# val-iisc/Reflecting-Reality

Hardware: AMD Instinct MI355X
Metric: images/sec at 512x512, 50-step DDIM, SD1.5+BrushNet (higher is better)
Workload: dtype bf16; 1 GPU; SD1.5 + BrushNet(6 cond ch) depth-cond inpaint, batch 4x512x512 per GPU, 50-step DDIM, CFG 7.5, VAE encode+decode included, random-init weights, inputs resident on the device; per_gpu_batch=4, global_batch=4, height=512, width=512, denoise_steps=50, parallelism=batch-shard x1 (no collective)

## Files before the change

reflecting-reality_amd/csrc/gemm_conv_kernel.h:

```cpp
#pragma once
#include "mf_common.h"

#include <type_traits>

#ifndef MF_XTAP
#define MF_XTAP 1
#endif
#ifndef MF_AEARLY
#define MF_AEARLY 1
#endif

namespace mfgemm {

static __device__ __attribute__((aligned(16))) unsigned int g_zero_page[16];

#ifdef MF_STAMPS
#define MF_STAMP(slot) do { if (p.stamps) { const int t_ = (int)threadIdx.x; \
    if (t_ == 0) p.stamps[(size_t)blockIdx.x * 32 + (slot)] = __builtin_amdgcn_s_memrealtime(); \
    else if (t_ == (int)blockDim.x - 256) p.stamps[(size_t)blockIdx.x * 32 + 16 + (slot)] = __builtin_amdgcn_s_memrealtime(); } } while (0)
#define MF_STAMP_DRAIN() asm volatile("s_waitcnt vmcnt(0)" ::: "memory")
#define MF_CLK(v) const unsigned long long v = __builtin_amdgcn_s_memtime()
#define MF_SUM(acc, a, b) acc += (b) - (a)
#define MF_PUT(slot, v) do { if (p.stamps) { const int t_ = (int)threadIdx.x; \
    if (t_ == 0) p.stamps[(size_t)blockIdx.x * 32 + (slot)] = (v); \
    else if (t_ == (int)blockDim.x - 256) p.stamps[(size_t)blockIdx.x * 32 + 16 + (slot)] = (v); } } while (0)
#else
#define MF_STAMP(slot) do { } while (0)
#define MF_STAMP_DRAIN() do { } while (0)
#define MF_CLK(v) do { } while (0)
#define MF_SUM(acc, a, b) do { } while (0)
#define MF_PUT(slot, v) do { } while (0)
#endif

struct GemmArgs {
    const char* a0; const char* a1;
    int C0, Ctot;
    int ld0b, ld1b;
    int Hin, Win, Ho, Wo, HoWo, KW, stride, pad_t, pad_l, ups;
    const char* w; int64_t ldw;
    int M, N, K;
    int zdiv; int64_t a_zs_o, a_zs_i, w_zs_o, w_zs_i, o_zs_o, o_zs_i;
    int splitk, kt_per_split, nkt, nz;
    float* ws;
    unsigned* sk_tickets;
    const float* bias; int bias_mode;
    const float* rs; const float* cs; int64_t rs_zs, cs_zs;
    const float* temb; int64_t ld_temb;
    const char* res0; int res0_dt; int64_t ld_res0;
    const char* res1; int res1_dt; int64_t ld_res1;
    int res1_rows;
    float alpha; int act;
    char* out; int out_dt; int64_t ldc;
    int tiles_n, tiles_m, ord_mfast, ord_pw, nblk, vec_ok, fast, dbg_no_res_pre;
    int dbg_epi;
    int pointwise;
    int howo_sh, wo_sh, ho_sh;
    unsigned wfr_magic;
    int epb;
    int epb_sh;
    unsigned* ovf;
    unsigned long long* stamps;
    const float* ln_cs; float ln_eps;
    char* vt_out; int vt_n0, vt_tokens; int64_t vt_ld;
    int nloop;
    float2* gn_part;
    float2* gn_grp; int gn_cpg;
};

__device__ __forceinline__ int div_sh(int x, int d, int sh) { return sh >= 0 ? x >> sh : x / d; }

__device__ __forceinline__ int res1_row(const GemmArgs& p, int m) {
    if (p.res1_rows > 0)
        while (m >= p.res1_rows) m -= p.res1_rows;
    return m;
}

__device__ __forceinline__ void epilogue_store(const GemmArgs& p, int64_t zo, int m, int n, float v, int zq = 0) {
    if (p.rs) v *= p.rs[zq * p.rs_zs + m];
    if (p.cs) v *= p.cs[zq * p.cs_zs + n];
    if (p.bias) v += p.bias_mode ? p.bias[m] : p.bias[n];
    if (p.temb) v += p.temb[(int64_t)div_sh(m, p.HoWo, p.howo_sh) * p.ld_temb + n];
    v *= p.alpha;
    if (p.res0) v += load_as_f32(p.res0, p.res0_dt, (int64_t)m * p.ld_res0 + n);
    if (p.res1) v += load_as_f32(p.res1, p.res1_dt, (int64_t)res1_row(p, m) * p.ld_res1 + n);
    if (p.act == MF_ACT_SILU) v = silu_precise(v);
    store_from_f32(p.out, p.out_dt, zo + (int64_t)m * p.ldc + n, v);
}

template <bool F16 = false>
__device__ __forceinline__ void load8_as_f32(const char* p, int dt, int64_t idx, float* o) {
    if (dt == MF_F32) {
        const float4 a = *reinterpret_cast<const float4*>(p + idx * 4);
        const float4 b = *reinterpret_cast<const float4*>(p + idx * 4 + 16);
        o[0] = a.x; o[1] = a.y; o[2] = a.z; o[3] = a.w; o[4] = b.x; o[5] = b.y; o[6] = b.z; o[7] = b.w;
    } else {
        unpack_h8<F16>(*reinterpret_cast<const uint4*>(p + idx * 2), o);
    }
}

__device__ __forceinline__ void unpack8_bf16(const uint4& u, float* o) {
    o[0] = __uint_as_float(u.x << 16); o[1] = __uint_as_float(u.x & 0xffff0000u);
    o[2] = __uint_as_float(u.y << 16); o[3] = __uint_as_float(u.y & 0xffff0000u);
    o[4] = __uint_as_float(u.z << 16); o[5] = __uint_as_float(u.z & 0xffff0000u);
    o[6] = __uint_as_float(u.w << 16); o[7] = __uint_as_float(u.w & 0xffff0000u);
}

template <bool F16>
__device__ __forceinline__ void epilogue_store8(const GemmArgs& p, int64_t zo, int m, int n, float* v, bool pre = false,
                                                const uint4& q0 = uint4{0, 0, 0, 0}, const uint4& q1 = uint4{0, 0, 0, 0}, int zq = 0,
                                                const char* eb = nullptr, const char* et = nullptr) {
    if (p.rs || p.cs) {
        const float r = p.rs ? p.rs[zq * p.rs_zs + m] : 1.0f;
        float c8[8] = {1, 1, 1, 1, 1, 1, 1, 1};
        if (p.cs) load8_as_f32((const char*)(p.cs + zq * p.cs_zs), MF_F32, n, c8);
#pragma unroll
        for (int j = 0; j < 8; ++j) v[j] *= r * c8[j];
    }
    if (p.bias) {
        if (p.bias_mode) {
            const float b = p.bias[m];
#pragma unroll
            for (int j = 0; j < 8; ++j) v[j] += b;
        } else {
            float b[8];
            if (eb) load8_as_f32(eb, MF_F32, 0, b);
            else load8_as_f32((const char*)p.bias, MF_F32, n, b);
#pragma unroll
            for (int j = 0; j < 8; ++j) v[j] += b[j];
        }
    }
    if (p.temb) {
        float t[8];
        if (et) load8_as_f32(et, MF_F32, 0, t);
        else load8_as_f32((const char*)p.temb, MF_F32, (int64_t)div_sh(m, p.HoWo, p.howo_sh) * p.ld_temb + n, t);
#pragma unroll
        for (int j = 0; j < 8; ++j) v[j] += t[j];
    }
#pragma unroll
    for (int j = 0; j < 8; ++j) v[j] *= p.alpha;
    if (p.res0) {
        float r[8];
        if (pre) unpack_h8<F16>(q0, r);
        else load8_as_f32<F16>(p.res0, p.res0_dt, (int64_t)m * p.ld_res0 + n, r);
#pragma unroll
        for (int j = 0; j < 8; ++j) v[j] += r[j];
    }
    if (p.res1) {
        float r[8];
        if (pre) unpack_h8<F16>(q1, r);
        else load8_as_f32<F16>(p.res1, p.res1_dt, (int64_t)res1_row(p, m) * p.ld_res1 + n, r);
#pragma unroll
        for (int j = 0; j < 8; ++j) v[j] += r[j];
    }
    if (p.act == MF_ACT_SILU) {
#pragma unroll
        for (int j = 0; j < 8; ++j) v[j] = silu_precise(v[j]);
    }
    if (p.act == MF_ACT_GEGLU4) {
        float g[4];
        if (p.out_dt != MF_F32) {
#pragma unroll
            for (int j = 0; j < 4; ++j) {
                const float x = v[4 + j];
                const float z = fabsf(x) * 0.70710678118654752440f;
                const float t = __builtin_amdgcn_rcpf(fmaf(0.3275911f, z, 1.0f));
                const float poly = t * fmaf(t, fmaf(t, fmaf(t, fmaf(t, 1.061405429f, -1.453152027f), 1.421413741f), -0.284496736f), 0.254829592f);
                const float e = 1.0f - poly * __builtin_amdgcn_exp2f(-z * z * 1.44269504088896340736f);
                g[j] = v[j] * (0.5f * x + 0.5f * fabsf(x) * e);
            }
        } else {
#pragma unroll
            for (int j = 0; j < 4; ++j) g[j] = v[j] * (0.5f * v[4 + j] * (1.0f + erff(v[4 + j] * 0.70710678118654752440f)));
        }
        const int64_t o = zo + (int64_t)m * p.ldc + (n >> 1);
        if (p.out_dt == MF_F32) {
            *reinterpret_cast<float4*>(p.out + o * 4) = make_float4(g[0], g[1], g[2], g[3]);
        } else {
            uint2 u;
            u.x = pack_h2<F16>(g[0], g[1]);
            u.y = pack_h2<F16>(g[2], g[3]);
            *reinterpret_cast<uint2*>(p.out + o * 2) = u;
        }
        return;
    }
    const int64_t o = zo + (int64_t)m * p.ldc + n;
    if (p.out_dt == MF_F32) {
        *reinterpret_cast<float4*>(p.out + o * 4) = make_float4(v[0], v[1], v[2], v[3]);
        *reinterpret_cast<float4*>(p.out + o * 4 + 16) = make_float4(v[4], v[5], v[6], v[7]);
    } else {
        *reinterpret_cast<uint4*>(p.out + o * 2) = pack_h8<F16>(v);
    }
}

__device__ __forceinline__ uint4 ld8f_to_bf16(const char* p) {
    const float4 lo = *reinterpret_cast<const float4*>(p);
    const float4 hi = *reinterpret_cast<const float4*>(p + 16);
    uint4 r;
    r.x = pack_bf16x2(lo.x, lo.y);
    r.y = pack_bf16x2(lo.z, lo.w);
    r.z = pack_bf16x2(hi.x, hi.y);
    r.w = pack_bf16x2(hi.z, hi.w);
    return r;
}

typedef __attribute__((address_space(1))) const void* gbl_ptr_t;

__device__ __forceinline__ void dma16(const char* src, char* lds_wave_base) {
    const unsigned lds_off = __builtin_amdgcn_readfirstlane((unsigned)(size_t)(lds_ptr_t)lds_wave_base);
    unsigned keep;
    asm volatile("s_mov_b32 %0, m0\n\ts_mov_b32 m0, %2\n\ts_nop 0\n\tglobal_load_lds_dwordx4 %1, off\n\ts_mov_b32 m0, %0"
                 : "=&s"(keep) : "v"(src), "s"(lds_off) : "memory");
}

template <int DT>
__device__ __forceinline__ f32x4_t mfma16x32(bf16x8_t a, bf16x8_t b, f32x4_t c, int, int, int) {
    if constexpr (DT == MF_F16) return __builtin_amdgcn_mfma_f32_16x16x32_f16(__builtin_bit_cast(f16x8_t, a), __builtin_bit_cast(f16x8_t, b), c, 0, 0, 0);
    else return __builtin_amdgcn_mfma_f32_16x16x32_bf16(a, b, c, 0, 0, 0);
}
template <int DT>
__device__ __forceinline__ f32x16_t mfma32x16(bf16x8_t a, bf16x8_t b, f32x16_t c) {
    if constexpr (DT == MF_F16) return __builtin_amdgcn_mfma_f32_32x32x16_f16(__builtin_bit_cast(f16x8_t, a), __builtin_bit_cast(f16x8_t, b), c, 0, 0, 0);
    else return __builtin_amdgcn_mfma_f32_32x32x16_bf16(a, b, c, 0, 0, 0);
}

#define MF_FX_XT 1
#define MF_FX_EPB 2
#define MF_FX_AE 4
#define MF_FX_ALL 7
#define MF_FX_XQ 8

constexpr int epb_pitch(int bn) { return (bn + 63) / 64 * 64; }
constexpr int epb_off(int bm, int bn, int stages, bool dx, bool ws) {
    return dx ? 2 * (bm + 32) * 128 + (ws ? stages : 2) * bn * 128 : stages * (bm + bn) * 128 + (ws ? bm * 8 : 0);
}
constexpr int epb_nimg(int bm, int bn, int stages, bool dx, bool ws) {
    if (!ws) return 0;
    const int room = 160 * 1024 - epb_off(bm, bn, stages, dx, ws), row = epb_pitch(bn) * 4;
    return room >= 6 * row ? 4 : (room >= 3 * row ? 1 : 0);
}

constexpr int min_waves(int bm, int bn, int stages, int nthr) {
    const int smem = stages * (bm + bn) * 128;
    int blocks = 160 * 1024 / smem;
    if (blocks > 8) blocks = 8;
    int w = blocks * (nthr / 64) / 4;
    return w < 1 ? 1 : (w > 4 ? 4 : w);
}

template <int BM, int BN, int NT_ALL, bool F16>
__device__ __forceinline__ void splitk_combine_tail(const GemmArgs& p, char* smem, int tile_m, int tile_n, int z, int zq, int64_t zo, int t) {
    asm volatile("s_waitcnt vmcnt(0)" ::: "memory");
    __syncthreads();
    unsigned* last_flag = reinterpret_cast<unsigned*>(smem);
    if (t == 0) {
        __builtin_amdgcn_fence(__ATOMIC_RELEASE, "agent");
        asm volatile("s_waitcnt vmcnt(0)" ::: "memory");
        unsigned* tk = p.sk_tickets + ((int64_t)z * p.tiles_m + tile_m) * p.tiles_n + tile_n;
        const unsigned prev = __hip_atomic_fetch_add(tk, 1u, __ATOMIC_RELAXED, __HIP_MEMORY_SCOPE_AGENT);
        const bool last = prev == (unsigned)p.splitk - 1u;
        if (last) {
            __hip_atomic_store(tk, 0u, __ATOMIC_RELAXED, __HIP_MEMORY_SCOPE_AGENT);
            __builtin_amdgcn_fence(__ATOMIC_ACQUIRE, "agent");
            asm volatile("s_waitcnt vmcnt(0)" ::: "memory");
        }
        *last_flag = last ? 1u : 0u;
    }
    __syncthreads();
    if (*last_flag == 0u) return;
    const int m0 = tile_m * BM, n0 = tile_n * BN;
    constexpr int CPR = BN / 8;
    const int64_t mn = (int64_t)p.M * p.N;
    const bool vec = p.vec_ok && (p.N & 3) == 0;
    for (int it = t; it < BM * CPR; it += NT_ALL) {
        const int row = it / CPR, ec = (it - row * CPR) * 8;
        const int m = m0 + row, n = n0 + ec;
        if (m >= p.M || n >= p.N) continue;
        const float* src = p.ws + (int64_t)z * mn + (int64_t)m * p.N + n;
        if (vec && n + 8 <= p.N) {
            float v[8] = {0, 0, 0, 0, 0, 0, 0, 0};
            for (int s = 0; s < p.splitk; ++s) {
                const float4 a = *reinterpret_cast<const float4*>(src + (int64_t)s * p.nz * mn);
                const float4 b = *reinterpret_cast<const float4*>(src + (int64_t)s * p.nz * mn + 4);
                v[0] += a.x; v[1] += a.y; v[2] += a.z; v[3] += a.w; v[4] += b.x; v[5] += b.y; v[6] += b.z; v[7] += b.w;
            }
            epilogue_store8<F16>(p, zo, m, n, v, false, uint4{0, 0, 0, 0}, uint4{0, 0, 0, 0}, zq);
        } else {
            for (int jj = 0; jj < 8 && n + jj < p.N; ++jj) {
                float v = 0.0f;
                for (int s = 0; s < p.splitk; ++s) v += src[(int64_t)s * p.nz * mn + jj];
                epilogue_store(p, zo, m, n + jj, v, zq);
            }
        }
    }
}

template <int DT, int BM, int BN, int WAVES_M, int WAVES_N, bool A_F32, int STAGES, bool DXR = false, bool WPK = false, bool M16 = false,
          bool WS = false, bool P16 = false, bool SKF = false, int FX = 0>
__global__ __launch_bounds__(WAVES_M* WAVES_N * 64 + (WS ? 256 : 0),
                             WS ? (WAVES_M * WAVES_N + 4) / 4 : min_waves(BM + (DXR ? 32 : 0), BN, STAGES, WAVES_M* WAVES_N * 64))
void gemm_conv_kernel(const GemmArgs p) {
    constexpr int NTHR = WAVES_M * WAVES_N * 64;
    constexpr int NSTG = WS ? 256 : NTHR;
    constexpr bool H16 = DT == MF_BF16 || DT == MF_F16;
    static_assert(!WS || ((H16 || (DT == MF_F16X3 && WPK && !M16 && !P16)) && !A_F32 && STAGES == 3),
                  "warp specialisation: bf16 / fp16 (or the parity mode with a pre-split W), LDS-DMA staging, 3-deep ring");
    static_assert(!M16 || (H16 && !A_F32), "the 16x16x32 form is instantiated for bf16 / fp16 only");
    constexpr bool X1 = DT == MF_BF16X1;
    constexpr bool SPLIT = (DT == MF_F16X3 || DT == MF_BF16X3 || X1);
    static_assert(!WPK || (SPLIT && !X1), "a pre-split W operand only exists for the three-MFMA split codes");
    constexpr bool FP8 = (DT == MF_FP8);
    constexpr int ES = H16 ? 2 : (FP8 ? 1 : 4);
    constexpr int AES = A_F32 ? 4 : ES;
    constexpr int VEC = 16 / ES;
    constexpr int BK = 128 / ES;
    constexpr int WM = BM / WAVES_M, WN = BN / WAVES_N;
    static_assert(!P16 || (H16 && !M16 && !A_F32 && (WM == 32 || WM == 64) && WN % 16 == 0), "P16: 16-bit operands, 32- or 64-row wave tiles");
    constexpr int MT = WM / 32, NT = P16 ? 1 : WN / 32;
    constexpr int MT16 = WM / 16, NT16 = WN / 16;
    constexpr int RPP = NSTG / 8;
    constexpr int A_IT = BM / RPP, B_IT = BN / RPP;
    constexpr int STAGE_BYTES = (BM + BN) * 128;
    constexpr int EP_RS = (WN + 4) * 4;
    static_assert(WM % 32 == 0 && (P16 || WN % 32 == 0), "wave tile must be a multiple of 32x32");
    static_assert(BM % RPP == 0 && BN % RPP == 0, "tile rows must be a multiple of the staging pass");
    constexpr int SR = (WAVES_M * WAVES_N * 32 * EP_RS <= STAGES * STAGE_BYTES) ? 32 : 16;
    static_assert(WAVES_M * WAVES_N * SR * EP_RS <= STAGES * STAGE_BYTES, "epilogue slabs must fit in the staging LDS");
    static_assert(STAGES >= 2 && STAGES <= 6, "2 to 6 LDS stages");
    static_assert(!A_F32 || STAGES == 2, "the register-staged path is double buffered");
    static_assert(!A_F32 || DT == MF_BF16, "A_F32 only converts fp32 activations for bf16 compute");

    extern __shared__ __attribute__((aligned(16))) char smem[];
    MF_STAMP(0);

    const bool producer = WS && __builtin_amdgcn_readfirstlane((int)threadIdx.x) >= NTHR;
    const int tid = producer ? (int)threadIdx.x - NTHR : (int)threadIdx.x;
    const int lane = tid & 63;
    const int wave = __builtin_amdgcn_readfirstlane(tid >> 6);
    const int wm = wave / WAVES_N, wn = wave % WAVES_N;
    if constexpr (WS) {
        if ((p.dbg_epi & 16) && !producer) __builtin_amdgcn_s_setprio(1);
        if ((p.dbg_epi & 32) && producer) __builtin_amdgcn_s_setprio(1);
    }

    int bid = blockIdx.x;
// ... 818 lines not shown
                    st_c = st_c == STAGES - 1 ? 0 : st_c + 1;
                    st_i = st_i == STAGES - 1 ? 0 : st_i + 1;
                }
            };
            auto ring_ws = [&](auto issue) {
                if (producer) {
                    int st_i = 0, issued = 0;
                    auto issue_next = [&]() { issue(st_i); st_i = st_i == STAGES - 1 ? 0 : st_i + 1; ++issued; };
                    auto wait_for = [&](int need) {
                        const int newer = issued - 1 - need;
                        static_assert((PF - 1) * G < 64, "vmcnt is a 6-bit counter");
                        if (PF >= 3 && newer >= 2) wait_vmcnt<2 * G>();
                        else if (PF >= 2 && newer == 1) wait_vmcnt<G>();
                        else wait_vmcnt<0>();
                    };
                    const bool lnf = p.ln_cs != nullptr;
                    float ln_s[A_IT], ln_q[A_IT];
#pragma unroll
                    for (int i = 0; i < A_IT; ++i) { ln_s[i] = 0.0f; ln_q[i] = 0.0f; }
                    int st_s = 0;
                    auto ln_tile = [&]() {
                        if constexpr (DT == MF_BF16) {
                            typedef __attribute__((ext_vector_type(2))) __bf16 bf2_t;
                            const bf2_t ones = __builtin_bit_cast(bf2_t, 0x3F803F80u);
                            const char* As = smem + st_s * STAGE_BYTES + tid * 16;
#pragma unroll
                            for (int i = 0; i < A_IT; ++i) {
                                const uint4 u = *reinterpret_cast<const uint4*>(As + i * RPP * 128);
                                const unsigned w4[4] = {u.x, u.y, u.z, u.w};
#pragma unroll
                                for (int e = 0; e < 4; ++e) {
                                    const bf2_t v = __builtin_bit_cast(bf2_t, w4[e]);
                                    ln_s[i] = __builtin_amdgcn_fdot2_f32_bf16(v, ones, ln_s[i], false);
                                    ln_q[i] = __builtin_amdgcn_fdot2_f32_bf16(v, v, ln_q[i], false);
                                }
                            }
                        } else if constexpr (DT == MF_F16) {
                            const char* As = smem + st_s * STAGE_BYTES + tid * 16;
#pragma unroll
                            for (int i = 0; i < A_IT; ++i) {
                                const uint4 u = *reinterpret_cast<const uint4*>(As + i * RPP * 128);
                                const unsigned w4[4] = {u.x, u.y, u.z, u.w};
#pragma unroll
                                for (int e = 0; e < 4; ++e) {
                                    const mf_f16x2_t v = __builtin_bit_cast(mf_f16x2_t, w4[e]);
                                    const float a0 = (float)v[0], a1 = (float)v[1];
                                    ln_s[i] += a0 + a1;
                                    ln_q[i] = fmaf(a0, a0, fmaf(a1, a1, ln_q[i]));
                                }
                            }
                        }
                        st_s = st_s == STAGES - 1 ? 0 : st_s + 1;
                    };
                    for (int k = 0; k < PF && k < nt; ++k) issue_next();
                    wait_for(0);
                    __builtin_amdgcn_s_barrier();
                    MF_STAMP(2);
                    [[maybe_unused]] unsigned long long w_iss = 0, w_vm = 0, w_bar = 0;
                    for (int t = 0; t + 1 < nt; ++t) {
                        MF_CLK(c0);
                        if (t + PF < nt) issue_next();
                        if (lnf) ln_tile();
                        MF_CLK(c1);
                        wait_for(t + 1);
                        MF_CLK(c2);
                        __builtin_amdgcn_s_barrier();
                        MF_CLK(c3);
                        MF_SUM(w_iss, c0, c1); MF_SUM(w_vm, c1, c2); MF_SUM(w_bar, c2, c3);
                    }
                    MF_PUT(13, w_vm); MF_PUT(14, w_bar); MF_PUT(15, w_iss);
                    if (lnf) {
                        ln_tile();
                        float2* lnst = reinterpret_cast<float2*>(smem + STAGES * STAGE_BYTES);
                        const float invk = 1.0f / (float)p.K;
#pragma unroll
                        for (int i = 0; i < A_IT; ++i) {
                            float s1 = ln_s[i], q1 = ln_q[i];
#pragma unroll
                            for (int off = 1; off < 8; off <<= 1) {
                                s1 += __shfl_xor(s1, off, 64);
                                q1 += __shfl_xor(q1, off, 64);
                            }
                            const float mean = s1 * invk;
                            float var = q1 * invk - mean * mean;
                            if (var < 0.0f) var = 0.0f;
                            if ((tid & 7) == 0) lnst[lrow + i * RPP] = make_float2(mean, 1.0f / sqrtf(var + p.ln_eps));
                        }
                    }
                } else {
                    int st_c = 0;
                    __builtin_amdgcn_s_barrier();
                    MF_STAMP(2);
                    if constexpr (XT) {
                        const int arb = wm * WM + ((P16 || M16) ? r16 : frow);
                        auto ld = [&](auto S, auto P) {
                            const char* Ab = smem + st_c * STAGE_BYTES;
                            const char* Bb = Ab + BM * 128 + (wn * WN + ((P16 || M16) ? r16 : frow)) * 128;
                            if constexpr (P16 || M16) xt_load(S, P, Ab, [&](int t) { return arb + t * 16; }, Bb);
                            else xt_load(S, P, Ab, [&](int i) { return arb + i * 32; }, Bb);
                        };
                        xt_loop(ld, [&]() { st_c = st_c == STAGES - 1 ? 0 : st_c + 1; });
                    } else
                    for (int t = 0; t < nt; ++t) {
                        compute(st_c);
                        st_c = st_c == STAGES - 1 ? 0 : st_c + 1;
                        if (t + 1 < nt) __builtin_amdgcn_s_barrier();
                    }
                }
            };
            if constexpr (WS) {
                if (p.fast) {
                    if (producer) fast_init();
                    ring_ws(issue_tile_fast);
                } else {
                    ring_ws(issue_tile);
                }
            } else if (p.fast) {
                fast_init();
                ring(issue_tile_fast);
            } else {
                ring(issue_tile);
            }
        } else {
            load_tile_regs();
            store_tile_regs(0);
            if (nt > 1) load_tile_regs();
            __syncthreads();
            for (int t = 0; t < nt; ++t) {
                compute(t & 1);
                if (t + 1 < nt) {
                    store_tile_regs((t + 1) & 1);
                    if (t + 2 < nt) load_tile_regs();
                }
                __syncthreads();
            }
        }
    }
    MF_STAMP(3);
    if constexpr (EPB_NIMG > 0) {
        if (producer && epb) wait_vmcnt<0>();
    }
    __syncthreads();
    MF_STAMP(4);
    if constexpr (DT == MF_F16X3) mf_raise_if_over(p.ovf, split_amax);

    char* slab = smem + wave * (SR * EP_RS);
    constexpr int CPR = WN / 8;
    constexpr int ITEMS = SR * CPR;
    float* ws = p.splitk > 1 ? p.ws + ((int64_t)ksplit * p.nz + z) * (int64_t)p.M * p.N : nullptr;
    const int64_t zo = zq * p.o_zs_o + zr * p.o_zs_i;
    const bool res_pre = !ws && p.vec_ok && (p.res0 || p.res1) && (!p.res0 || p.res0_dt != MF_F32) &&
                         (!p.res1 || p.res1_dt != MF_F32) && !p.dbg_no_res_pre;
    constexpr int NIT = (ITEMS + 63) / 64;
    if constexpr (WS) {
        constexpr int NCW = WAVES_M * WAVES_N, TW = NCW + 4, NCHUNK = NCW * NIT, MAXC = (NCHUNK + TW - 1) / TW;
        const int g = producer ? NCW + wave : wave;
        const bool gn = p.gn_part != nullptr;
        constexpr int GNP = (NCW * WN + TW * 64 - 1) / (TW * 64);
        float gns[GNP], gnq[GNP];
#pragma unroll
        for (int k = 0; k < GNP; ++k) { gns[k] = 0.0f; gnq[k] = 0.0f; }
#pragma unroll
        for (int ih = 0; ih < MT * (32 / SR); ++ih) {
            const int i = ih / (32 / SR), half = ih % (32 / SR);
            uint4 q0[MAXC], q1[MAXC];
            auto coords = [&](int u, int& sw, int& row, int& ec, int& m, int& n) -> bool {
                const int c = g + u * TW;
                sw = c / NIT;
                const int it = (c - sw * NIT) * 64 + lane;
                row = it / CPR; ec = (it - row * CPR) * 8;
                const int swm = sw / WAVES_N, swn = sw - swm * WAVES_N;
                m = m0 + swm * WM + i * 32 + half * SR + row;
                n = n0 + swn * WN + ec;
                return c < NCHUNK && (ITEMS % 64 == 0 || it < ITEMS);
            };
            if (res_pre) {
#pragma unroll
                for (int u = 0; u < MAXC; ++u) {
                    int sw, row, ec, m, n;
                    const bool on = coords(u, sw, row, ec, m, n);
                    q0[u] = uint4{0, 0, 0, 0}; q1[u] = uint4{0, 0, 0, 0};
                    if (on && m < p.M && n + 8 <= p.N) {
                        if (p.res0) q0[u] = *reinterpret_cast<const uint4*>(p.res0 + ((int64_t)m * p.ld_res0 + n) * 2);
                        if (p.res1) q1[u] = *reinterpret_cast<const uint4*>(p.res1 + ((int64_t)res1_row(p, m) * p.ld_res1 + n) * 2);
                    }
                }
            }
            if (!producer) {
                if constexpr (P16) {
#pragma unroll
                    for (int a = 0; a < 2; ++a)
#pragma unroll
                        for (int b = 0; b < NT16; ++b)
#pragma unroll
                            for (int r = 0; r < 4; ++r) {
                                const int row = 16 * a + 4 * kg + r - half * SR;
                                if (SR == 32 || a == half)
                                    *reinterpret_cast<float*>(slab + row * EP_RS + (16 * b + r16) * 4) = acc16[2 * i + a][b][r];
                            }
                } else {
#pragma unroll
                    for (int j = 0; j < NT; ++j)
#pragma unroll
                        for (int e = half * (SR / 2); e < half * (SR / 2) + SR / 2; ++e) {
                            if constexpr (M16) {
                                const int row = 16 * (e >> 3) + 4 * kg + (e & 3) - half * SR;
                                *reinterpret_cast<float*>(slab + row * EP_RS + (j * 32 + 16 * ((e >> 2) & 1) + r16) * 4) = acc[i][j][e];
                            } else {
                                const int row = (e & 3) + 8 * (e >> 2) + 4 * fh - half * SR;
                                *reinterpret_cast<float*>(slab + row * EP_RS + (j * 32 + frow) * 4) = acc[i][j][e];
                            }
                        }
                }
            }
            MF_STAMP(7 + 3 * ih);
            __builtin_amdgcn_s_waitcnt(0xc07f);
            __builtin_amdgcn_s_barrier();
            MF_STAMP(8 + 3 * ih);
#pragma unroll
            for (int u = 0; u < MAXC; ++u) {
                int sw, row, ec, m, n;
                if (!coords(u, sw, row, ec, m, n)) continue;
                const char* sl = smem + sw * (SR * EP_RS);
                const float2* lnst = reinterpret_cast<const float2*>(smem + STAGES * STAGE_BYTES);
                if (p.vt_out && n0 + (sw % WAVES_N) * WN >= p.vt_n0) {
                    static_assert(SR % 8 == 0 && (SR / 8) * WN == ITEMS, "transposed items cover the slab");
                    const int c = g + u * TW, it = (c - sw * NIT) * 64 + lane;
                    const int rg = it % (SR / 8), col = it / (SR / 8);
                    const int swm = sw / WAVES_N, swn = sw - swm * WAVES_N;
                    const int mt = m0 + swm * WM + i * 32 + half * SR + rg * 8, nt_ = n0 + swn * WN + col;
                    if (mt < p.M && nt_ < p.N) {
                        float tv[8];
#pragma unroll
                        for (int j = 0; j < 8; ++j) tv[j] = *reinterpret_cast<const float*>(sl + (rg * 8 + j) * EP_RS + col * 4);
                        const char* erow = smem + EPB_OFF + (nt_ - n0) * 4;
                        if (p.ln_cs) {
                            const float cs = epb ? *reinterpret_cast<const float*>(erow + EPB_PITCH * 4) : p.ln_cs[nt_];
#pragma unroll
                            for (int j = 0; j < 8; ++j) {
                                const float2 st = lnst[mt - m0 + j];
                                tv[j] = st.y * (tv[j] - st.x * cs);
                            }
                        }
                        const float b = p.bias ? (epb ? *reinterpret_cast<const float*>(erow) : p.bias[nt_]) : 0.0f;
#pragma unroll
                        for (int j = 0; j < 8; ++j) tv[j] = (tv[j] + b) * p.alpha;
                        const int img = mt / p.vt_tokens, tok = mt - img * p.vt_tokens;
                        const uint4 o = pack_h8<DT == MF_F16>(tv);
                        *reinterpret_cast<uint4*>(p.vt_out + (((int64_t)img * (p.N - p.vt_n0) + (nt_ - p.vt_n0)) * p.vt_ld + tok) * 2) = o;
                    }
                    continue;
                }
                float v[8];
                float4 lo, hi;
#ifdef MF_STAMPS
                if (p.dbg_epi & 2) { lo = make_float4(1.0f, 2.0f, 3.0f, (float)u); hi = lo; } else
#endif
                {
                    lo = *reinterpret_cast<const float4*>(sl + row * EP_RS + ec * 4);
                    hi = *reinterpret_cast<const float4*>(sl + row * EP_RS + ec * 4 + 16);
                }
#ifdef MF_STAMPS
                if (p.dbg_epi & 1) { asm volatile("" ::"v"(lo.x), "v"(hi.w)); continue; }
#endif
                if (p.ln_cs && m < p.M && n + 8 <= p.N) {
                    const float2 st = lnst[m - m0];
                    const float* lc = epb ? reinterpret_cast<const float*>(smem + EPB_OFF + (EPB_PITCH + n - n0) * 4) : p.ln_cs + n;
                    const float4 c0 = *reinterpret_cast<const float4*>(lc);
                    const float4 c1 = *reinterpret_cast<const float4*>(lc + 4);
                    lo.x = st.y * (lo.x - st.x * c0.x); lo.y = st.y * (lo.y - st.x * c0.y);
                    lo.z = st.y * (lo.z - st.x * c0.z); lo.w = st.y * (lo.w - st.x * c0.w);
                    hi.x = st.y * (hi.x - st.x * c1.x); hi.y = st.y * (hi.y - st.x * c1.y);
                    hi.z = st.y * (hi.z - st.x * c1.z); hi.w = st.y * (hi.w - st.x * c1.w);
                }
                v[0] = lo.x; v[1] = lo.y; v[2] = lo.z; v[3] = lo.w; v[4] = hi.x; v[5] = hi.y; v[6] = hi.z; v[7] = hi.w;
                if (m < p.M && n < p.N) {
                    if (ws) {
                        if (n + 8 <= p.N && (p.N & 3) == 0) {
                            *reinterpret_cast<float4*>(ws + (int64_t)m * p.N + n) = lo;
                            *reinterpret_cast<float4*>(ws + (int64_t)m * p.N + n + 4) = hi;
                        } else {
                            for (int jj = 0; jj < 8 && n + jj < p.N; ++jj) ws[(int64_t)m * p.N + n + jj] = v[jj];
                        }
                    } else if (p.vec_ok && n + 8 <= p.N) {
                        if (epb) {
                            const char* eb = smem + EPB_OFF + (n - n0) * 4;
                            epilogue_store8<DT == MF_F16>(p, zo, m, n, v, res_pre, q0[u], q1[u], zq, eb, eb + (2 + (m >> p.epb_sh) - (m0 >> p.epb_sh)) * (EPB_PITCH * 4));
                        } else {
                            epilogue_store8<DT == MF_F16>(p, zo, m, n, v, res_pre, q0[u], q1[u], zq);
                        }
                        if (gn) {
                            char* slw = smem + sw * (SR * EP_RS) + row * EP_RS + ec * 4;
                            *reinterpret_cast<float4*>(slw) = make_float4(v[0], v[1], v[2], v[3]);
                            *reinterpret_cast<float4*>(slw + 16) = make_float4(v[4], v[5], v[6], v[7]);
                        }
                    } else {
                        for (int jj = 0; jj < 8 && n + jj < p.N; ++jj) epilogue_store(p, zo, m, n + jj, v[jj], zq);
                    }
                }
            }
            MF_STAMP(9 + 3 * ih);
            if (gn) {
                __builtin_amdgcn_s_waitcnt(0xc07f);
                __builtin_amdgcn_s_barrier();
#pragma unroll
                for (int k = 0; k < GNP; ++k) {
                    const int pid = (g + k * TW) * 64 + lane;
                    if (pid < NCW * WN) {
                        const int sw = pid / WN, col = pid - sw * WN;
                        const char* sl = smem + sw * (SR * EP_RS) + col * 4;
                        float a = 0.0f, b = 0.0f;
#pragma unroll
                        for (int r = 0; r < SR; ++r) {
                            const float x = *reinterpret_cast<const float*>(sl + r * EP_RS);
                            a += x; b = fmaf(x, x, b);
                        }
                        gns[k] += a; gnq[k] += b;
                    }
                }
            }
            if (ih + 1 < MT * (32 / SR) || gn) {
                __builtin_amdgcn_s_waitcnt(0xc07f);
                __builtin_amdgcn_s_barrier();
            }
        }
        if (gn) {
            float2* red = reinterpret_cast<float2*>(smem);
#pragma unroll
            for (int k = 0; k < GNP; ++k) {
                const int pid = (g + k * TW) * 64 + lane;
                if (pid < NCW * WN) {
                    const int sw = pid / WN, col = pid - sw * WN;
                    const int swm = sw / WAVES_N, swn = sw - swm * WAVES_N;
                    red[swm * BN + swn * WN + col] = make_float2(gns[k], gnq[k]);
                }
            }
            __builtin_amdgcn_s_waitcnt(0xc07f);
            __builtin_amdgcn_s_barrier();
            const int tcol = (int)threadIdx.x;
            float a = 0.0f, b = 0.0f;
            if (tcol < BN && n0 + tcol < p.N) {
#pragma unroll
                for (int w2 = 0; w2 < WAVES_M; ++w2) { const float2 x = red[w2 * BN + tcol]; a += x.x; b += x.y; }
                p.gn_part[(int64_t)tile_m * p.N + n0 + tcol] = make_float2(a, b);
            }
            if (p.gn_grp) {
                float2* tot = red + WAVES_M * BN;
                if (tcol < BN) tot[tcol] = make_float2(a, b);
                __builtin_amdgcn_s_waitcnt(0xc07f);
                __builtin_amdgcn_s_barrier();
                const int cpg = p.gn_cpg, c0g = tcol * cpg;
                if (c0g < BN && n0 + c0g < p.N) {
                    float ga = 0.0f, gb = 0.0f;
                    for (int j = 0; j < cpg; ++j) { const float2 x = tot[c0g + j]; ga += x.x; gb += x.y; }
                    p.gn_grp[(int64_t)tile_m * (p.N / cpg) + (n0 + c0g) / cpg] = make_float2(ga, gb);
                }
            }
        }
        MF_STAMP_DRAIN();
        MF_STAMP(5);
        if constexpr (SKF) {
            if (ws) splitk_combine_tail<BM, BN, NTHR + 256, DT == MF_F16>(p, smem, tile_m, tile_n, z, zq, zo, (int)threadIdx.x);
        }
        MF_STAMP(6);
        return;
    }
    const bool gn = p.gn_part != nullptr;
    constexpr int GNC = (WN + 63) / 64;
    float gns[GNC], gnq[GNC];
#pragma unroll
    for (int k = 0; k < GNC; ++k) { gns[k] = 0.0f; gnq[k] = 0.0f; }
#pragma unroll
    for (int ih = 0; ih < MT * (32 / SR); ++ih) {
        const int i = ih / (32 / SR), half = ih % (32 / SR);
        uint4 q0[NIT], q1[NIT];
        if (res_pre) {
#pragma unroll
            for (int k = 0; k < NIT; ++k) {
                const int it = k * 64 + lane;
                const int row = it / CPR, ec = (it - row * CPR) * 8;
                const int m = m0 + wm * WM + i * 32 + half * SR + row;
                const int n = n0 + wn * WN + ec;
                q0[k] = uint4{0, 0, 0, 0}; q1[k] = uint4{0, 0, 0, 0};
                if ((ITEMS % 64 == 0 || it < ITEMS) && m < p.M && n + 8 <= p.N) {
                    if (p.res0) q0[k] = *reinterpret_cast<const uint4*>(p.res0 + ((int64_t)m * p.ld_res0 + n) * 2);
                    if (p.res1) q1[k] = *reinterpret_cast<const uint4*>(p.res1 + ((int64_t)res1_row(p, m) * p.ld_res1 + n) * 2);
                }
            }
        }
        if constexpr (P16) {
#pragma unroll
            for (int a = 0; a < 2; ++a)
#pragma unroll
                for (int b = 0; b < NT16; ++b)
#pragma unroll
                    for (int r = 0; r < 4; ++r) {
                        const int row = 16 * a + 4 * kg + r - half * SR;
                        if (SR == 32 || a == half)
                            *reinterpret_cast<float*>(slab + row * EP_RS + (16 * b + r16) * 4) = acc16[2 * i + a][b][r];
                    }
        } else
#pragma unroll
        for (int j = 0; j < NT; ++j)
#pragma unroll
            for (int e = half * (SR / 2); e < half * (SR / 2) + SR / 2; ++e) {
                if constexpr (M16) {
                    const int row = 16 * (e >> 3) + 4 * kg + (e & 3) - half * SR;
                    *reinterpret_cast<float*>(slab + row * EP_RS + (j * 32 + 16 * ((e >> 2) & 1) + r16) * 4) = acc[i][j][e];
                } else {
                    const int row = (e & 3) + 8 * (e >> 2) + 4 * fh - half * SR;
                    *reinterpret_cast<float*>(slab + row * EP_RS + (j * 32 + frow) * 4) = acc[i][j][e];
                }
            }
        __builtin_amdgcn_s_waitcnt(0xc07f);
        __builtin_amdgcn_wave_barrier();
#pragma unroll
        for (int it0 = 0; it0 < ITEMS; it0 += 64) {
            const int it = it0 + lane;
            if (ITEMS % 64 != 0 && it >= ITEMS) continue;
            const int row = it / CPR, ec = (it - row * CPR) * 8;
            const int m = m0 + wm * WM + i * 32 + half * SR + row;
            const int n = n0 + wn * WN + ec;
            float v[8];
            const float4 lo = *reinterpret_cast<const float4*>(slab + row * EP_RS + ec * 4);
            const float4 hi = *reinterpret_cast<const float4*>(slab + row * EP_RS + ec * 4 + 16);
            v[0] = lo.x; v[1] = lo.y; v[2] = lo.z; v[3] = lo.w; v[4] = hi.x; v[5] = hi.y; v[6] = hi.z; v[7] = hi.w;
            if (m < p.M && n < p.N) {
                if (ws) {
                    if (n + 8 <= p.N && (p.N & 3) == 0) {
                        *reinterpret_cast<float4*>(ws + (int64_t)m * p.N + n) = lo;
                        *reinterpret_cast<float4*>(ws + (int64_t)m * p.N + n + 4) = hi;
                    } else {
                        for (int jj = 0; jj < 8 && n + jj < p.N; ++jj) ws[(int64_t)m * p.N + n + jj] = v[jj];
                    }
                } else if (p.vec_ok && n + 8 <= p.N) {
                    epilogue_store8<DT == MF_F16>(p, zo, m, n, v, res_pre, q0[it0 / 64], q1[it0 / 64], zq);
                    if (gn) {
                        *reinterpret_cast<float4*>(slab + row * EP_RS + ec * 4) = make_float4(v[0], v[1], v[2], v[3]);
                        *reinterpret_cast<float4*>(slab + row * EP_RS + ec * 4 + 16) = make_float4(v[4], v[5], v[6], v[7]);
                    }
                } else {
                    for (int jj = 0; jj < 8 && n + jj < p.N; ++jj) epilogue_store(p, zo, m, n + jj, v[jj], zq);
                }
            }
        }
        __builtin_amdgcn_s_waitcnt(0xc07f);
        __builtin_amdgcn_wave_barrier();
        if (gn) {
#pragma unroll
            for (int k = 0; k < GNC; ++k) {
                const int col = lane + 64 * k;
                if (WN % 64 == 0 || col < WN) {
                    float a = 0.0f, b = 0.0f;
#pragma unroll
                    for (int r = 0; r < SR; ++r) {
                        const float x = *reinterpret_cast<const float*>(slab + r * EP_RS + col * 4);
                        a += x; b = fmaf(x, x, b);
                    }
                    gns[k] += a; gnq[k] += b;
                }
            }
            __builtin_amdgcn_s_waitcnt(0xc07f);
            __builtin_amdgcn_wave_barrier();
        }
    }
    if (gn) {
        __syncthreads();
        float2* red = reinterpret_cast<float2*>(smem);
#pragma unroll
        for (int k = 0; k < GNC; ++k) {
            const int col = lane + 64 * k;
            if (WN % 64 == 0 || col < WN) red[wm * BN + wn * WN + col] = make_float2(gns[k], gnq[k]);
        }
        __syncthreads();
        float2* tot = red + WAVES_M * BN;
        for (int tcol = (int)threadIdx.x; tcol < BN; tcol += NTHR) {
            float a = 0.0f, b = 0.0f;
            if (n0 + tcol < p.N) {
#pragma unroll
                for (int w2 = 0; w2 < WAVES_M; ++w2) { const float2 x = red[w2 * BN + tcol]; a += x.x; b += x.y; }
                p.gn_part[(int64_t)tile_m * p.N + n0 + tcol] = make_float2(a, b);
            }
            if (p.gn_grp) tot[tcol] = make_float2(a, b);
        }
        if (p.gn_grp) {
            __syncthreads();
            const int cpg = p.gn_cpg;
            for (int c0g = (int)threadIdx.x * cpg; c0g < BN; c0g += NTHR * cpg) {
                if (n0 + c0g < p.N) {
                    float ga = 0.0f, gb = 0.0f;
                    for (int j = 0; j < cpg; ++j) { const float2 x = tot[c0g + j]; ga += x.x; gb += x.y; }
                    p.gn_grp[(int64_t)tile_m * (p.N / cpg) + (n0 + c0g) / cpg] = make_float2(ga, gb);
                }
            }
        }
    }
    MF_STAMP_DRAIN();
    MF_STAMP(5);
    if constexpr (SKF) {
        if (ws) splitk_combine_tail<BM, BN, NTHR, DT == MF_F16>(p, smem, tile_m, tile_n, z, zq, zo, (int)threadIdx.x);
    }
    MF_STAMP(6);
}

template <int DT, int BM, int BN, int WMv, int WNv, bool AF, int ST, bool DX = false, bool WPK = false, bool M16 = false, bool WS = false,
          bool P16 = false, bool SKF = false, int FX = 0>
void launch_one(const GemmArgs& a, dim3 grid, hipStream_t s) {
    constexpr int smem_k = DX ? 2 * (BM + (WS ? 32 : WMv * WNv * 8)) * 128 + (WS ? ST : 2) * BN * 128 : ST * (BM + BN) * 128 + (WS ? BM * 8 : 0);
    constexpr int smem_e = (FX & MF_FX_EPB) && epb_nimg(BM, BN, ST, DX, WS) > 0 ? (2 + epb_nimg(BM, BN, ST, DX, WS)) * epb_pitch(BN) * 4 : 0;
    static_assert(smem_k == epb_off(BM, BN, ST, DX, WS) || !WS, "epb_off must equal the ring's footprint");
    static_assert(smem_k + smem_e <= 160 * 1024, "LDS");
    static const int smem_min = getenv("MFHIP_SMEM_MIN") ? atoi(getenv("MFHIP_SMEM_MIN")) : 0;
    const int smem = smem_k + smem_e > smem_min ? smem_k + smem_e : smem_min;
    static bool attr_set = false;
    if (!attr_set) {
        (void)hipFuncSetAttribute(reinterpret_cast<const void*>(&gemm_conv_kernel<DT, BM, BN, WMv, WNv, AF, ST, DX, WPK, M16, WS, P16, SKF, FX>),
                                  hipFuncAttributeMaxDynamicSharedMemorySize, smem);
        attr_set = true;
    }
    hipLaunchKernelGGL((gemm_conv_kernel<DT, BM, BN, WMv, WNv, AF, ST, DX, WPK, M16, WS, P16, SKF, FX>), grid, dim3(WMv * WNv * 64 + (WS ? 256 : 0)), smem, s, a);
}

template <int DT, int BM, int BN, int WMv, int WNv, bool AF, int ST, bool DX = false, bool WPK = false, bool M16 = false, bool WS = false,
          bool P16 = false, int FX = 0>
void launch_skf(const GemmArgs& a, dim3 grid, hipStream_t s) {
    if (a.sk_tickets) launch_one<DT, BM, BN, WMv, WNv, AF, ST, DX, WPK, M16, WS, P16, true, FX>(a, grid, s);
    else launch_one<DT, BM, BN, WMv, WNv, AF, ST, DX, WPK, M16, WS, P16, false, FX>(a, grid, s);
}

bool launch_nloop(int dtype, const GemmArgs& a, hipStream_t s);
bool launch_pers(int dtype, const GemmArgs& a, hipStream_t s);
bool launch_bf16_a(int tile, const GemmArgs& a, dim3 grid, hipStream_t s, bool a_f32);
bool launch_bf16_b(int tile, const GemmArgs& a, dim3 grid, hipStream_t s);
bool launch_bf16_c(int tile, const GemmArgs& a, dim3 grid, hipStream_t s);
bool launch_bf16_ws_dx(int tile, const GemmArgs& a, dim3 grid, hipStream_t s);
bool launch_bf16_ws_ring(int tile, const GemmArgs& a, dim3 grid, hipStream_t s);
bool launch_f16_a(int tile, const GemmArgs& a, dim3 grid, hipStream_t s, bool a_f32);
bool launch_f16_b(int tile, const GemmArgs& a, dim3 grid, hipStream_t s);
bool launch_f16_c(int tile, const GemmArgs& a, dim3 grid, hipStream_t s);
bool launch_f16_ws_dx(int tile, const GemmArgs& a, dim3 grid, hipStream_t s);
bool launch_f16_ws_ring(int tile, const GemmArgs& a, dim3 grid, hipStream_t s);
bool launch_f32_a(int tile, const GemmArgs& a, dim3 grid, hipStream_t s);
bool launch_f32_b(int tile, const GemmArgs& a, dim3 grid, hipStream_t s);
bool launch_f16x3(int tile, const GemmArgs& a, dim3 grid, hipStream_t s, bool wpk);
bool launch_f16x3_ws(int tile, const GemmArgs& a, dim3 grid, hipStream_t s);
bool launch_bf16x3(int tile, const GemmArgs& a, dim3 grid, hipStream_t s, bool wpk);
bool launch_bf16x1(int tile, const GemmArgs& a, dim3 grid, hipStream_t s);
bool launch_fp8(int tile, const GemmArgs& a, dim3 grid, hipStream_t s);
bool launch_halo_family(int tile, const GemmArgs& a, dim3 grid, hipStream_t s);

}
```

Measured before the change: 5.210 images/sec.

## Add specialized fast epilogue with LDS-staged bias/temb rows for warp-specialized GEMM

Adds a compile-time specialized epilogue path for half-precision warp-specialized GEMM/conv tiles. Bias and timestep-embedding rows are staged once into spare LDS, and each 8-wide output item then does vectorized bias/temb/residual/alpha/SiLU math and a packed store, replacing the per-element generic epilogue. The path is chosen at runtime (three template modes: generic, fast, fast with residual preload) and can be forced off through an environment variable. It adds code size and register pressure from the extra instantiated variants, and relies on the LDS budget arithmetic being correct.

```diff
diff --git a/reflecting-reality_amd/csrc/gemm_conv_kernel.h b/reflecting-reality_amd/csrc/gemm_conv_kernel.h
--- a/reflecting-reality_amd/csrc/gemm_conv_kernel.h
+++ b/reflecting-reality_amd/csrc/gemm_conv_kernel.h
@@ -65,6 +65,7 @@
     int nloop;
     float2* gn_part;
     float2* gn_grp; int gn_cpg;
+    int dbg_generic_epi;
 };
 
 __device__ __forceinline__ int div_sh(int x, int d, int sh) { return sh >= 0 ? x >> sh : x / d; }
@@ -190,6 +191,34 @@
     } else {
         *reinterpret_cast<uint4*>(p.out + o * 2) = pack_h8<F16>(v);
     }
+}
+
+template <bool F16>
+__device__ __forceinline__ void epilogue_item16(const GemmArgs& p, char* out, float* v, bool has_b, const char* eb, bool has_t, const char* et,
+                                                bool has_r0, bool has_r1, const uint4& q0, const uint4& q1) {
+    if (has_b) {
+        const float4 a = *reinterpret_cast<const float4*>(eb), b = *reinterpret_cast<const float4*>(eb + 16);
+        v[0] += a.x; v[1] += a.y; v[2] += a.z; v[3] += a.w; v[4] += b.x; v[5] += b.y; v[6] += b.z; v[7] += b.w;
+    }
+    if (has_t) {
+        const float4 a = *reinterpret_cast<const float4*>(et), b = *reinterpret_cast<const float4*>(et + 16);
+        v[0] += a.x; v[1] += a.y; v[2] += a.z; v[3] += a.w; v[4] += b.x; v[5] += b.y; v[6] += b.z; v[7] += b.w;
+    }
+    float r0[8], r1[8];
+    unpack_h8<F16>(q0, r0);
+    unpack_h8<F16>(q1, r1);
+#pragma unroll
+    for (int j = 0; j < 8; ++j) {
+        float x = v[j] * p.alpha;
+        x = has_r0 ? x + r0[j] : x;
+        x = has_r1 ? x + r1[j] : x;
+        v[j] = x;
+    }
+    if (p.act == MF_ACT_SILU) {
+#pragma unroll
+        for (int j = 0; j < 8; ++j) v[j] = silu_precise(v[j]);
+    }
+    *reinterpret_cast<uint4*>(out) = pack_h8<F16>(v);
 }
 
 __device__ __forceinline__ uint4 ld8f_to_bf16(const char* p) {
@@ -1314,6 +1343,59 @@
     const bool res_pre = !ws && p.vec_ok && (p.res0 || p.res1) && (!p.res0 || p.res0_dt != MF_F32) &&
                          (!p.res1 || p.res1_dt != MF_F32) && !p.dbg_no_res_pre;
     constexpr int NIT = (ITEMS + 63) / 64;
+    constexpr int FR_OFF = WAVES_M * WAVES_N * SR * EP_RS;
+    constexpr int FR_LDS = WS ? epb_off(BM, BN, STAGES, DXR, WS) : (DXR ? 2 * (BM + 32) * 128 + 2 * BN * 128 : STAGES * STAGE_BYTES);
+    constexpr int FR_ROOM = (FR_LDS - FR_OFF) / (BN * 4);
+    constexpr int FR_NIMG = FR_ROOM >= 5 ? 4 : (FR_ROOM >= 1 ? FR_ROOM - 1 : -1);
+    constexpr int FR_THR = NTHR + (WS ? 256 : 0);
+    constexpr int FR_IT = FR_NIMG >= 0 ? ((1 + FR_NIMG) * BN + FR_THR - 1) / FR_THR : 1;
+    constexpr bool FAST_EPI = H16 && WS && !(BM == 256 && BN == 160) && !(DXR && P16 && BM == 128 && WAVES_M == 4);
+    bool fastp = false, fr_stage = false;
+    int fr_img0 = 0, fr_nimg = 0;
+    if constexpr (FAST_EPI) {
+        fastp = !p.dbg_generic_epi && !ws && p.vec_ok && p.out_dt != MF_F32 && !p.rs && !p.cs && p.bias_mode == 0 &&
+                (p.act == MF_ACT_NONE || p.act == MF_ACT_SILU) && !p.ln_cs && !p.vt_out && ((!p.res0 && !p.res1) || res_pre);
+        if (fastp && !epb && (p.bias || p.temb)) {
+            if (p.temb) {
+                const int mlast = (m0 + BM < p.M ? m0 + BM : p.M) - 1;
+                fr_img0 = div_sh(m0, p.HoWo, p.howo_sh);
+                fr_nimg = div_sh(mlast, p.HoWo, p.howo_sh) - fr_img0 + 1;
+            }
+            fr_stage = fr_nimg <= FR_NIMG;
+            fastp = fr_stage;
+        }
+    }
+    auto fr_load = [&](float* fr_v) {
+        if constexpr (FR_NIMG >= 0) {
+            if (fr_stage) {
+#pragma unroll
+                for (int k = 0; k < FR_IT; ++k) {
+                    const int idx = k * FR_THR + (int)threadIdx.x;
+                    const int r = idx / BN, n = n0 + idx - r * BN;
+                    const float* src = r == 0 ? p.bias : (p.temb ? p.temb + (int64_t)(fr_img0 + r - 1) * p.ld_temb : nullptr);
+                    const bool on = r <= fr_nimg && n < p.N && src != nullptr;
+                    fr_v[k] = on ? src[n] : 0.0f;
+                }
+            }
+        }
+    };
+    auto fr_publish = [&](const float* fr_v) {
+        if constexpr (FR_NIMG >= 0) {
+            if (fr_stage) {
+#pragma unroll
+                for (int k = 0; k < FR_IT; ++k) {
+                    const int idx = k * FR_THR + (int)threadIdx.x;
+                    if (idx < (1 + FR_NIMG) * BN) *reinterpret_cast<float*>(smem + FR_OFF + idx * 4) = fr_v[k];
+                }
+            }
+        }
+    };
+    const bool fr_bias = p.bias != nullptr, fr_temb = p.temb != nullptr;
+    auto fr_rows = [&](int m, int n, int& eb, int& et) {
+        const int img = fr_temb ? (epb ? (m >> p.epb_sh) - (m0 >> p.epb_sh) : div_sh(m, p.HoWo, p.howo_sh) - fr_img0) : 0;
+        eb = (epb ? EPB_OFF : FR_OFF) + (n - n0) * 4;
+        et = eb + (epb ? (2 + img) * (EPB_PITCH * 4) : (1 + img) * (BN * 4));
+    };
     if constexpr (WS) {
         constexpr int NCW = WAVES_M * WAVES_N, TW = NCW + 4, NCHUNK = NCW * NIT, MAXC = (NCHUNK + TW - 1) / TW;
         const int g = producer ? NCW + wave : wave;
@@ -1322,10 +1404,16 @@
         float gns[GNP], gnq[GNP];
 #pragma unroll
         for (int k = 0; k < GNP; ++k) { gns[k] = 0.0f; gnq[k] = 0.0f; }
+        auto rounds = [&](auto MODE_) {
+        constexpr int MODE = decltype(MODE_)::value;
 #pragma unroll
         for (int ih = 0; ih < MT * (32 / SR); ++ih) {
             const int i = ih / (32 / SR), half = ih % (32 / SR);
             uint4 q0[MAXC], q1[MAXC];
+            float fr_v[FR_IT];
+            if constexpr (MODE != 0) {
+                if (ih == 0) fr_load(fr_v);
+            }
             auto coords = [&](int u, int& sw, int& row, int& ec, int& m, int& n) -> bool {
                 const int c = g + u * TW;
                 sw = c / NIT;
@@ -1336,7 +1424,7 @@
                 n = n0 + swn * WN + ec;
                 return c < NCHUNK && (ITEMS % 64 == 0 || it < ITEMS);
             };
-            if (res_pre) {
+            if (MODE == 2 || (MODE == 0 && res_pre)) {
 #pragma unroll
                 for (int u = 0; u < MAXC; ++u) {
                     int sw, row, ec, m, n;
@@ -1375,10 +1463,40 @@
                         }
                 }
             }
+            if constexpr (MODE != 0) {
+                if (ih == 0) fr_publish(fr_v);
+            }
             MF_STAMP(7 + 3 * ih);
             __builtin_amdgcn_s_waitcnt(0xc07f);
             __builtin_amdgcn_s_barrier();
             MF_STAMP(8 + 3 * ih);
+            if constexpr (MODE != 0) {
+                if constexpr (MODE == 2) {
+                    asm volatile("s_waitcnt vmcnt(0)" ::: "memory");
+#pragma unroll
+                    for (int u = 0; u < MAXC; ++u)
+                        asm volatile("" : "+v"(q0[u].x), "+v"(q0[u].y), "+v"(q0[u].z), "+v"(q0[u].w), "+v"(q1[u].x), "+v"(q1[u].y), "+v"(q1[u].z), "+v"(q1[u].w));
+                }
+                const bool has_r0 = MODE == 2 && p.res0 != nullptr, has_r1 = MODE == 2 && p.res1 != nullptr;
+#pragma unroll
+                for (int u = 0; u < MAXC; ++u) {
+                    int sw, row, ec, m, n;
+                    if (!coords(u, sw, row, ec, m, n)) continue;
+                    if (m < p.M && n < p.N) {
+                        char* slw = smem + sw * (SR * EP_RS) + row * EP_RS + ec * 4;
+                        const float4 lo = *reinterpret_cast<const float4*>(slw), hi = *reinterpret_cast<const float4*>(slw + 16);
+                        float v[8] = {lo.x, lo.y, lo.z, lo.w, hi.x, hi.y, hi.z, hi.w};
+                        int eb, et;
+                        fr_rows(m, n, eb, et);
+                        epilogue_item16<DT == MF_F16>(p, p.out + (zo + (int64_t)m * p.ldc + n) * 2, v, fr_bias, smem + eb, fr_temb, smem + et,
+                                                      has_r0, has_r1, q0[u], q1[u]);
+                        if (gn) {
+                            *reinterpret_cast<float4*>(slw) = make_float4(v[0], v[1], v[2], v[3]);
+                            *reinterpret_cast<float4*>(slw + 16) = make_float4(v[4], v[5], v[6], v[7]);
+                        }
+                    }
+                }
+            } else
 #pragma unroll
             for (int u = 0; u < MAXC; ++u) {
                 int sw, row, ec, m, n;
@@ -1486,6 +1604,14 @@
                 __builtin_amdgcn_s_barrier();
             }
         }
+        };
+        if constexpr (FAST_EPI) {
+            if (!fastp) rounds(std::integral_constant<int, 0>{});
+            else if (res_pre) rounds(std::integral_constant<int, 2>{});
+            else rounds(std::integral_constant<int, 1>{});
+        } else {
+            rounds(std::integral_constant<int, 0>{});
+        }
         if (gn) {
             float2* red = reinterpret_cast<float2*>(smem);
 #pragma unroll
@@ -1665,6 +1791,11 @@
     MF_STAMP(6);
 }
 
+inline int generic_epi_forced() {
+    const char* e = getenv("MFHIP_GENERIC_EPI");
+    return e != nullptr && e[0] != '\0' && e[0] != '0';
+}
+
 template <int DT, int BM, int BN, int WMv, int WNv, bool AF, int ST, bool DX = false, bool WPK = false, bool M16 = false, bool WS = false,
           bool P16 = false, bool SKF = false, int FX = 0>
 void launch_one(const GemmArgs& a, dim3 grid, hipStream_t s) {
@@ -1680,7 +1811,9 @@
                                   hipFuncAttributeMaxDynamicSharedMemorySize, smem);
         attr_set = true;
     }
-    hipLaunchKernelGGL((gemm_conv_kernel<DT, BM, BN, WMv, WNv, AF, ST, DX, WPK, M16, WS, P16, SKF, FX>), grid, dim3(WMv * WNv * 64 + (WS ? 256 : 0)), smem, s, a);
+    GemmArgs b = a;
+    b.dbg_generic_epi = generic_epi_forced();
+    hipLaunchKernelGGL((gemm_conv_kernel<DT, BM, BN, WMv, WNv, AF, ST, DX, WPK, M16, WS, P16, SKF, FX>), grid, dim3(WMv * WNv * 64 + (WS ? 256 : 0)), smem, s, b);
 }
 
 template <int DT, int BM, int BN, int WMv, int WNv, bool AF, int ST, bool DX = false, bool WPK = false, bool M16 = false, bool WS = false,
```

Result: no change. 5.239 images/sec, median of 6 (+0.5%).
